# LuaAndC/lua-mapreduce-1

Hardware: AMD Instinct MI355X
Metric: words/sec (whole node), Europarl-v7 word-count 197 splits, 1/2/4/8 MI355X (higher is better)
Workload: dtype int64; 1 GPU; model=wordcount (MapReduce: taskfn/mapfn/partitionfn/reducefn), global_batch=197, seq_len=10000, parallelism=dp1, num_reducers=10, words=49158635, bytes=291393897, valid=True, input=host-staged-every-step

## Files before the change

csrc/hip/wordcount3.hip:

```cpp
#include <hip/hip_runtime.h>
#include "mr_common.h"
#include "hashtab.h"

MR_LONG_MASK_SYMBOL(wc3)

namespace mr {
namespace v3 {

constexpr int SEG = 16;
constexpr int PAD = 16;
constexpr int HALO = 64;
constexpr int PROBES = 32;

template <int T, int SLOTS>
struct Lds {
  static constexpr int TILE = T * SEG;
  static constexpr int STAGED = TILE + HALO;
  static constexpr int TXT = PAD + STAGED + 32;
  static constexpr int WSW = STAGED / 32 + 2;
  static constexpr int MAXTOK = T * 4;
  u8 txt[TXT];
  u32 ws[WSW];
  u16 tokpos[MAXTOK];
  u32 wsum[T / 64];
  u32 tnext;
  u64 tag[SLOTS];
  u32 cnt[SLOTS];
  u32 rep[SLOTS];
  u64 lo[SLOTS];
  u64 hi[SLOTS];
  u32 nclaimed;
};

struct Ovf {
  u64* hi;
  u64* lo;
  u64* rep;
  u64 cap;
  unsigned long long* counter;
};

__device__ __forceinline__ u32 ws_mask_word(u32 w) {
  u32 m = 0;
#pragma unroll
  for (int j = 0; j < 4; ++j) m |= (is_ws((w >> (8 * j)) & 0xFFu) ? 1u : 0u) << j;
  return m;
}

__device__ __forceinline__ u32 ws_mask16(uint4 q) {
  return ws_mask_word(q.x) | (ws_mask_word(q.y) << 4) | (ws_mask_word(q.z) << 8) | (ws_mask_word(q.w) << 12);
}

__device__ __forceinline__ u32 funnel(u32 a, u32 b, u32 r8) { return r8 ? ((a >> r8) | (b << (32 - r8))) : a; }

__device__ u64 long_lo_global(const u8* text, u64 p0, u64 len) {
  u64 h = long_hash_init(len);
  for (u64 w = 0; w < len; w += 8) {
    const u64 n = (len - w) < 8 ? (len - w) : 8;
    const u64 word = load_word_le(text + p0 + w, n);
    h = long_hash_step(h, word);
  }
  return long_lo(h, mr_long_mask);
}

__device__ __forceinline__ uint4 load16(const u8* __restrict__ text, u64 gpos, u64 nbytes, int aligned) {
  if (aligned && gpos + SEG <= nbytes) {
    typedef u32 v4u __attribute__((ext_vector_type(4)));
    const v4u v = __builtin_nontemporal_load(reinterpret_cast<const v4u*>(text + gpos));
    return make_uint4(v.x, v.y, v.z, v.w);
  }
  u32 w[4];
#pragma unroll
  for (int k = 0; k < 4; ++k) {
    w[k] = 0;
#pragma unroll
    for (int j = 0; j < 4; ++j) {
      const u64 p = gpos + 4 * k + j;
      w[k] |= (p < nbytes ? (u32)text[p] : 32u) << (8 * j);
    }
  }
  return make_uint4(w[0], w[1], w[2], w[3]);
}

template <int T, int SLOTS>
__device__ __forceinline__ bool lds_insert(Lds<T, SLOTS>& L, u64 hi, u64 lo, u32 rep, const u8* kb) {
  u64 h = hi ^ (lo * 0x9E3779B97F4A7C15ull);
  h ^= h >> 31;
  h *= 0xC2B2AE3D27D4EB4Full;
  h ^= h >> 29;
  const bool exact = (lo - 1 < 7) && (hi & 0xFFull) == 0;
  const u64 tag = exact ? (hi | lo) : ((h & ~0xFFull) | 0x80ull);
  u32 slot = (u32)(h >> 40) & (SLOTS - 1);
  constexpr u32 LIMIT = SLOTS * 3 / 4;
  for (int probes = 0; probes < PROBES;) {
    u64 cur = __hip_atomic_load(&L.tag[slot], __ATOMIC_RELAXED, __HIP_MEMORY_SCOPE_WORKGROUP);
    if (cur == 0) {
      if (__hip_atomic_load(&L.nclaimed, __ATOMIC_RELAXED, __HIP_MEMORY_SCOPE_WORKGROUP) >= LIMIT) return false;
      u64 expected = 0;
      if (__hip_atomic_compare_exchange_strong(&L.tag[slot], &expected, tag, __ATOMIC_RELAXED, __ATOMIC_RELAXED,
                                               __HIP_MEMORY_SCOPE_WORKGROUP)) {
        L.hi[slot] = hi;
        L.rep[slot] = rep;
        __hip_atomic_fetch_add(&L.cnt[slot], 1u, __ATOMIC_RELAXED, __HIP_MEMORY_SCOPE_WORKGROUP);
        __hip_atomic_fetch_add(&L.nclaimed, 1u, __ATOMIC_RELAXED, __HIP_MEMORY_SCOPE_WORKGROUP);
        if (exact) L.lo[slot] = lo;
        else __hip_atomic_store(&L.lo[slot], lo, __ATOMIC_RELEASE, __HIP_MEMORY_SCOPE_WORKGROUP);
        return true;
      }
      cur = expected;
    }
    if (cur == tag) {
      if (exact) {
        __hip_atomic_fetch_add(&L.cnt[slot], 1u, __ATOMIC_RELAXED, __HIP_MEMORY_SCOPE_WORKGROUP);
        return true;
      }
      const u64 l = __hip_atomic_load(&L.lo[slot], __ATOMIC_ACQUIRE, __HIP_MEMORY_SCOPE_WORKGROUP);
      if (l == 0) continue;
      if (l == lo && L.hi[slot] == hi &&
          (!key_is_long(lo) || rep_bytes_equal(kb, make_rep(L.rep[slot] & 0xFFFFu, L.rep[slot] >> 16),
                                               make_rep(rep & 0xFFFFu, rep >> 16)))) {
        __hip_atomic_fetch_add(&L.cnt[slot], 1u, __ATOMIC_RELAXED, __HIP_MEMORY_SCOPE_WORKGROUP);
        return true;
      }
    }
    slot = (slot + 1) & (SLOTS - 1);
    ++probes;
  }
  return false;
}

template <int T, int SLOTS, int TPC, bool STAMPS = false, bool DYN = false>
__global__ void __launch_bounds__(T) wc_map3_kernel(const u8* __restrict__ text, u64 nbytes, u64 rep_base, GTab g,
                                                    Ovf ovf, int aligned, u64* __restrict__ stamps = nullptr) {
  using L_t = Lds<T, SLOTS>;
  constexpr int TILE = L_t::TILE;
  constexpr int STAGED = L_t::STAGED;
  constexpr int WSW = L_t::WSW;
  constexpr u64 CHUNK = (u64)TILE * TPC;
  __shared__ __attribute__((aligned(16))) L_t L;
  const int t = threadIdx.x;
  const u64 chunk_begin = (u64)blockIdx.x * CHUNK;
  if (chunk_begin >= nbytes) return;
  const u64 chunk_end = min(chunk_begin + CHUNK, nbytes);
  [[maybe_unused]] u64 st_bar = 0, st_stage = 0, st_scan = 0, st_list = 0, st_loop = 0, st_flush = 0, st_p = 0;
  auto clk = [&]() -> u64 {
    if constexpr (STAMPS) return wall_clock64();
    return 0;
  };
  [[maybe_unused]] const u64 st_t0 = clk();
  auto bar = [&]() {
    const u64 a = clk();
    __syncthreads();
    if constexpr (STAMPS) st_bar += clk() - a;
  };
  for (int s = t; s < SLOTS; s += T) {
    L.tag[s] = 0;
    L.cnt[s] = 0;
    L.lo[s] = 0;
  }
  if (t == 0) {
    L.nclaimed = 0;
    L.txt[PAD - 1] = chunk_begin > 0 ? text[chunk_begin - 1] : (u8)' ';
    L.ws[WSW - 2] = 0xFFFFFFFFu;
    L.ws[WSW - 1] = 0xFFFFFFFFu;
  }
  u32 claims = 0;
  u16* ws16 = reinterpret_cast<u16*>(L.ws);
  const u32* txt32 = reinterpret_cast<const u32*>(L.txt);
  constexpr int NH = HALO / SEG;
  uint4 q = load16(text, chunk_begin + (u64)t * SEG, nbytes, aligned);
  uint4 qh = make_uint4(0, 0, 0, 0);
  if (t < NH) qh = load16(text, chunk_begin + TILE + (u64)t * SEG, nbytes, aligned);
  for (u64 tile_base = chunk_begin; tile_base < chunk_end; tile_base += TILE) {
    if (t == T - 1 && tile_base != chunk_begin) L.txt[PAD - 1] = L.txt[PAD + TILE - 1];
    bar();
    st_p = clk();
    *reinterpret_cast<uint4*>(L.txt + PAD + t * SEG) = q;
    ws16[t] = (u16)ws_mask16(q);
    if (t < NH) {
      *reinterpret_cast<uint4*>(L.txt + PAD + TILE + t * SEG) = qh;
      ws16[T + t] = (u16)ws_mask16(qh);
    }
    if constexpr (STAMPS) st_stage += clk() - st_p;
    bar();
    st_p = clk();
    const u64 next = tile_base + TILE;
    if (next < chunk_end) {
      q = load16(text, next + (u64)t * SEG, nbytes, aligned);
      if (t < NH) qh = load16(text, next + TILE + (u64)t * SEG, nbytes, aligned);
    }
    auto process = [&](u32 p) {
      u32 qq = p + 1;
      u32 wd = L.ws[qq >> 5] >> (qq & 31);
      u32 end;
      if (wd) {
        end = qq + __builtin_ctz(wd);
      } else {
        u32 k = (qq >> 5) + 1;
        while (L.ws[k] == 0) ++k;
        end = 32 * k + __builtin_ctz(L.ws[k]);
      }
      u64 len = end - p;
      const u64 gpos = tile_base + p;
      const u32 b = PAD + p;
      const u32 a = b >> 2;
      const u32 r8 = (b & 3u) * 8u;
      const u32 x0 = txt32[a], x1 = txt32[a + 1], x2 = txt32[a + 2], x3 = txt32[a + 3], x4 = txt32[a + 4];
      const u64 le_hi = (u64)funnel(x0, x1, r8) | ((u64)funnel(x1, x2, r8) << 32);
      const u64 le_lo = (u64)funnel(x2, x3, r8) | ((u64)funnel(x3, x4, r8) << 32);
      u64 hi = __builtin_bswap64(le_hi);
      u64 lo;
      if (end >= (u32)STAGED) {
        u64 pe = tile_base + STAGED;
        while (pe < nbytes && !is_ws(text[pe])) ++pe;
        len = pe - gpos;
      }
      if (len <= (u64)PACK_MAX) {
        if (len < 8) hi &= ~0ull << (8 * (8 - len));
        lo = len > 8 ? (__builtin_bswap64(le_lo) & (~0ull << (8 * (16 - len)))) : 0ull;
        lo |= len;
      } else {
        lo = long_lo_global(text, gpos, len);
      }
      const bool ok = len < 65536 && lds_insert(L, hi, lo, (u32)(gpos - chunk_begin) | ((u32)len << 16),
                                                 text + chunk_begin);
      if (!ok) {
        const u64 grep = make_rep(rep_base + gpos, len);
        const unsigned long long idx = atomicAdd(ovf.counter, 1ull);
        if (idx < ovf.cap) {
          ovf.hi[idx] = hi;
          ovf.lo[idx] = lo;
          ovf.rep[idx] = grep;
        } else {
          claims += gtab_insert(g, hi, lo, 1, grep, OP_SUM) == 2;
        }
      }
    };
    const u64 seg_base = tile_base + (u64)t * SEG;
    u32 starts = 0;
    if (seg_base < chunk_end) {
      const u32 m = ws16[t];
      const u32 prev_ws = t ? ((ws16[t - 1] >> 15) & 1u) : (is_ws(L.txt[PAD - 1]) ? 1u : 0u);
      starts = (~m) & ((m << 1) | prev_ws) & 0xFFFFu;
      const u64 lim_own = chunk_end - seg_base;
      if (lim_own < 16) starts &= (1u << lim_own) - 1u;
    }
    {
      constexpr int MAXTOK = L_t::MAXTOK;
      const int lane = t & 63, wave = t >> 6;
      const u32 c = __builtin_popcount(starts);
      u32 incl = c;
#pragma unroll
      for (int o = 1; o < 64; o <<= 1) {
        const u32 v = __shfl_up(incl, o);
        if (lane >= o) incl += v;
      }
      if (lane == 63) L.wsum[wave] = incl;
      if (DYN && t == 0) L.tnext = 0;
      if constexpr (STAMPS) st_scan += clk() - st_p;
      bar();
      st_p = clk();
      u32 base = 0, total = 0;
#pragma unroll
      for (int w = 0; w < T / 64; ++w) {
        const u32 x = L.wsum[w];
        base += w < wave ? x : 0u;
        total += x;
      }
      u32 k = base + incl - c;
      while (starts) {
        const int i = __builtin_ctz(starts);
        starts &= starts - 1;
        if (k < (u32)MAXTOK) L.tokpos[k] = (u16)(t * SEG + i);
        else process((u32)t * SEG + i);
        ++k;
      }
      if constexpr (STAMPS) st_list += clk() - st_p;
      bar();
      st_p = clk();
      const u32 ntok = total < (u32)MAXTOK ? total : (u32)MAXTOK;
      if constexpr (DYN) {
        for (;;) {
          u32 b0 = 0;
          if (lane == 0) b0 = __hip_atomic_fetch_add(&L.tnext, 64u, __ATOMIC_RELAXED, __HIP_MEMORY_SCOPE_WORKGROUP);
          b0 = __shfl(b0, 0);
          if (b0 >= ntok) break;
          if (b0 + lane < ntok) process(L.tokpos[b0 + lane]);
        }
      } else {
        for (u32 x = t; x < ntok; x += T) process(L.tokpos[x]);
      }
    }
    if constexpr (STAMPS) st_loop += clk() - st_p;
    bar();
  }
  [[maybe_unused]] const u64 st_f0 = clk();
  constexpr int PER = SLOTS / T;
  static_assert(SLOTS % T == 0, "slots must be a multiple of the block size");
  u64 khi[PER], klo[PER], ktag[PER], kslot[PER], gt[PER], gl[PER], gh[PER];
  u32 kcnt[PER], krep[PER];
#pragma unroll
  for (int k = 0; k < PER; ++k) {
    const int s = t + k * T;
    kcnt[k] = L.tag[s] != 0 ? L.cnt[s] : 0u;
    khi[k] = L.hi[s];
    klo[k] = L.lo[s];
    krep[k] = L.rep[s];
    ktag[k] = gtab_tag(khi[k], klo[k]);
    kslot[k] = gtab_home(ktag[k], g.mask);
  }
#pragma unroll
  for (int k = 0; k < PER; ++k) {
    if (kcnt[k]) {
      gt[k] = ld_agent(&g.s[kslot[k]].tag);
      if (!gtab_tag_exact(ktag[k])) {
        gl[k] = ld_agent(&g.s[kslot[k]].lo);
        gh[k] = ld_agent(&g.s[kslot[k]].hi);
      } else {
        gl[k] = klo[k];
        gh[k] = khi[k];
      }
    }
  }
  u32 state = 0;
#pragma unroll
  for (int k = 0; k < PER; ++k) {
    if (!kcnt[k]) {
      state |= 1u << k;
    } else if (gt[k] == ktag[k] && gl[k] == klo[k] && gh[k] == khi[k] && !key_is_long(klo[k])) {
      fold_value(&g.val[kslot[k]], (long long)kcnt[k], OP_SUM);
      state |= 1u << k;
    }
  }
  u32 won = 0;
#pragma unroll
  for (int k = 0; k < PER; ++k) {
    if (!(state & (1u << k)) && gt[k] == 0) {
      u64 expected = 0;
      if (__hip_atomic_compare_exchange_strong(&g.s[kslot[k]].tag, &expected, ktag[k], __ATOMIC_RELAXED,
                                               __ATOMIC_RELAXED, __HIP_MEMORY_SCOPE_AGENT))
        won |= 1u << k;
    }
  }
  if (won) {
#pragma unroll
    for (int k = 0; k < PER; ++k) {
      if (won & (1u << k)) {
        const u32 r = krep[k];
        st_agent(&g.s[kslot[k]].hi, khi[k]);
        st_agent(&g.s[kslot[k]].rep, make_rep(rep_base + chunk_begin + (r & 0xFFFFu), r >> 16));
        fold_value(&g.val[kslot[k]], (long long)kcnt[k], OP_SUM);
      }
    }
    asm volatile("s_waitcnt vmcnt(0)" ::: "memory");
#pragma unroll
    for (int k = 0; k < PER; ++k)
      if (won & (1u << k)) st_agent(&g.s[kslot[k]].lo, klo[k]);
    claims += __builtin_popcount(won);
    state |= won;
  }
#pragma unroll
  for (int k = 0; k < PER; ++k) {
    if (state & (1u << k)) continue;
    const u32 r = krep[k];
    claims += gtab_insert(g, khi[k], klo[k], (long long)kcnt[k],
                          make_rep(rep_base + chunk_begin + (r & 0xFFFFu), r >> 16), OP_SUM) == 2;
  }
  gtab_count_claims(g, claims);
  if constexpr (STAMPS) {
    const u64 now = clk();
    st_flush = now - st_f0;
    if ((t & 63) == 0) {
      u64* o = stamps + ((u64)blockIdx.x * (T / 64) + (t >> 6)) * 8;
      o[0] = now - st_t0;
      o[1] = st_bar;
      o[2] = st_stage;
      o[3] = st_scan;
      o[4] = st_list;
      o[5] = st_loop;
      o[6] = st_flush;
      o[7] = claims;
    }
  }
}

__global__ void __launch_bounds__(256) ovf_agg3_kernel(Ovf o, GTab g) {
  const unsigned long long n0 = *o.counter;
  const u64 n = n0 < o.cap ? n0 : o.cap;
  const u64 stride = (u64)gridDim.x * blockDim.x;
  u32 claims = 0;
  for (u64 i = (u64)blockIdx.x * blockDim.x + threadIdx.x; i < n; i += stride)
    claims += gtab_insert(g, o.hi[i], o.lo[i], 1ll, o.rep[i], OP_SUM) == 2;
  gtab_count_claims(g, claims);
}

constexpr int MAP_T = 512, MAP_SLOTS = 2048, MAP_TPC = 1;
static_assert(sizeof(Lds<MAP_T, MAP_SLOTS>) <= 80 * 1024, "two workgroups per CU");

static int g_map_dyn = 1;

template <int T, int SLOTS, int TPC>
static void launch_map3(const u8* text, u64 nbytes, u64 rep_base, const GTab& g, const Ovf& o, int aligned,
                        hipStream_t stream, u64* stamps = nullptr) {
  constexpr u64 CHUNK = (u64)T * SEG * TPC;
  const u64 nblocks = (nbytes + CHUNK - 1) / CHUNK;
  const dim3 grid((unsigned)nblocks), block(T);
  if (stamps && g_map_dyn)
    hipLaunchKernelGGL((wc_map3_kernel<T, SLOTS, TPC, true, true>), grid, block, 0, stream, text, nbytes, rep_base, g,
                       o, aligned, stamps);
  else if (stamps)
    hipLaunchKernelGGL((wc_map3_kernel<T, SLOTS, TPC, true>), grid, block, 0, stream, text, nbytes, rep_base, g, o,
                       aligned, stamps);
  else if (g_map_dyn)
    hipLaunchKernelGGL((wc_map3_kernel<T, SLOTS, TPC, false, true>), grid, block, 0, stream, text, nbytes, rep_base,
                       g, o, aligned, nullptr);
  else
    hipLaunchKernelGGL((wc_map3_kernel<T, SLOTS, TPC>), grid, block, 0, stream, text, nbytes, rep_base, g, o, aligned,
                       nullptr);
}

}
}

using namespace mr;

extern "C" {

int mr_wc3_set_dyn(int on) {
  v3::g_map_dyn = on ? 1 : 0;
  return 0;
}

int mr_wc_map3(const void* text, u64 nbytes, u64 rep_base, void* tag, void* hi, void* lo, void* val, void* rep,
               void* ctrl, u64 cap, void* ovf_hi, void* ovf_lo, void* ovf_rep, u64 ovf_cap, void* ovf_counter,
               hipStream_t stream) {
  if (nbytes == 0) return 0;
  (void)hi, (void)lo, (void)val;
  GTab g = gtab_make(tag, val, ctrl, cap, (const u8*)text - rep_base);
  v3::Ovf o{(u64*)ovf_hi, (u64*)ovf_lo, (u64*)ovf_rep, ovf_cap, (unsigned long long*)ovf_counter};
  const int aligned = ((uintptr_t)text & 15) == 0;
  const u8* t = (const u8*)text;
  v3::launch_map3<v3::MAP_T, v3::MAP_SLOTS, v3::MAP_TPC>(t, nbytes, rep_base, g, o, aligned, stream);
  hipLaunchKernelGGL(v3::ovf_agg3_kernel, dim3(1024), dim3(256), 0, stream, o, g);
  return (int)hipGetLastError();
}

int mr_wc_map3_stamped(const void* text, u64 nbytes, u64 rep_base, void* tag, void* val, void* ctrl, u64 cap,
                       void* ovf_hi, void* ovf_lo, void* ovf_rep, u64 ovf_cap, void* ovf_counter, void* stamps,
                       hipStream_t stream) {
  if (nbytes == 0 || stamps == nullptr) return nbytes ? -1 : 0;
  GTab g = gtab_make(tag, val, ctrl, cap, (const u8*)text - rep_base);
  v3::Ovf o{(u64*)ovf_hi, (u64*)ovf_lo, (u64*)ovf_rep, ovf_cap, (unsigned long long*)ovf_counter};
  const int aligned = ((uintptr_t)text & 15) == 0;
  v3::launch_map3<v3::MAP_T, v3::MAP_SLOTS, v3::MAP_TPC>((const u8*)text, nbytes, rep_base, g, o, aligned, stream,
                                                          (u64*)stamps);
  hipLaunchKernelGGL(v3::ovf_agg3_kernel, dim3(1024), dim3(256), 0, stream, o, g);
  return (int)hipGetLastError();
}

}
```

Before: 9.574 billion words/s.

## Streamline map kernel: SWAR whitespace mask, aligned loads, outlined cold paths

Replaces the per-byte whitespace test with a SWAR bit trick and always issues aligned 16-byte loads by shifting the base pointer back and blanking the leading and trailing bytes with spaces. Cold paths (long-token hashing, global insert, long-key compare) are moved into noinline functions, and the LDS insert is rewritten as a single-exit loop, both aimed at cutting register pressure and divergence. Short tokens now get their length from one alignbit of the whitespace bitmap. Exact-key slots store the key only in the tag, and token-list overflow is handled inside the processing loop. The aim is fewer instructions and VGPRs in the hot map loop, at the risk of call overhead and subtle edge-case bugs around the alignment lead.

```diff
diff --git a/csrc/hip/wordcount3.hip b/csrc/hip/wordcount3.hip
--- a/csrc/hip/wordcount3.hip
+++ b/csrc/hip/wordcount3.hip
@@ -41,10 +41,14 @@
 };
 
 __device__ __forceinline__ u32 ws_mask_word(u32 w) {
-  u32 m = 0;
-#pragma unroll
-  for (int j = 0; j < 4; ++j) m |= (is_ws((w >> (8 * j)) & 0xFFu) ? 1u : 0u) << j;
-  return m;
+  const u32 l7 = w & 0x7F7F7F7Fu;
+  const u32 ge9 = l7 + 0x77777777u;
+  const u32 ge14 = l7 + 0x72727272u;
+  const u32 ne32 = (l7 ^ 0x20202020u) + 0x7F7F7F7Fu;
+  u32 m = (((ge9 & ~ge14) | ~ne32) & ~w & 0x80808080u) >> 7;
+  m |= m >> 7;
+  m |= m >> 14;
+  return m & 0xFu;
 }
 
 __device__ __forceinline__ u32 ws_mask16(uint4 q) {
@@ -53,7 +57,7 @@
 
 __device__ __forceinline__ u32 funnel(u32 a, u32 b, u32 r8) { return r8 ? ((a >> r8) | (b << (32 - r8))) : a; }
 
-__device__ u64 long_lo_global(const u8* text, u64 p0, u64 len) {
+__device__ __noinline__ u64 long_lo_global(const u8* text, u64 p0, u64 len) {
   u64 h = long_hash_init(len);
   for (u64 w = 0; w < len; w += 8) {
     const u64 n = (len - w) < 8 ? (len - w) : 8;
@@ -63,23 +67,41 @@
   return long_lo(h, mr_long_mask);
 }
 
-__device__ __forceinline__ uint4 load16(const u8* __restrict__ text, u64 gpos, u64 nbytes, int aligned) {
-  if (aligned && gpos + SEG <= nbytes) {
-    typedef u32 v4u __attribute__((ext_vector_type(4)));
-    const v4u v = __builtin_nontemporal_load(reinterpret_cast<const v4u*>(text + gpos));
-    return make_uint4(v.x, v.y, v.z, v.w);
-  }
-  u32 w[4];
+__device__ __noinline__ u64 token_end_global(const u8* text, u64 pe, u64 end) {
+  while (pe < end && !is_ws(text[pe])) ++pe;
+  return pe;
+}
+
+__device__ __noinline__ bool lds_long_equal(const u8* kb, u32 ra, u32 rb) {
+  return rep_bytes_equal(kb, make_rep(ra & 0xFFFFu, ra >> 16), make_rep(rb & 0xFFFFu, rb >> 16));
+}
+
+__device__ __noinline__ u32 gtab_insert_sum(GTab g, u64 hi, u64 lo, u32 cnt, u64 rep) {
+  return gtab_insert(g, hi, lo, (long long)cnt, rep, OP_SUM) == 2;
+}
+
+__device__ __noinline__ uint4 space_out16(uint4 q, u32 from, u32 to) {
+  u32 w[4] = {q.x, q.y, q.z, q.w};
 #pragma unroll
   for (int k = 0; k < 4; ++k) {
-    w[k] = 0;
-#pragma unroll
-    for (int j = 0; j < 4; ++j) {
-      const u64 p = gpos + 4 * k + j;
-      w[k] |= (p < nbytes ? (u32)text[p] : 32u) << (8 * j);
-    }
+    u32 keep = 0;
+#pragma unroll
+    for (int j = 0; j < 4; ++j) keep |= ((u32)(4 * k + j) >= from && (u32)(4 * k + j) < to) ? 0xFFu << (8 * j) : 0u;
+    w[k] = (w[k] & keep) | (0x20202020u & ~keep);
   }
   return make_uint4(w[0], w[1], w[2], w[3]);
+}
+
+__device__ __forceinline__ uint4 load16(const u8* __restrict__ text, u64 g, u32 lead, u64 end) {
+  if (g >= end) return make_uint4(0x20202020u, 0x20202020u, 0x20202020u, 0x20202020u);
+  typedef u32 v4u __attribute__((ext_vector_type(4)));
+  const v4u v = __builtin_nontemporal_load(reinterpret_cast<const v4u*>(text + g));
+  uint4 q = make_uint4(v.x, v.y, v.z, v.w);
+  const u32 from = g == 0 ? lead : 0u;
+  const u64 left = end - g;
+  if (__builtin_expect(from != 0 || left < (u64)SEG, 0))
+    q = space_out16(q, from, left < (u64)SEG ? (u32)left : (u32)SEG);
+  return q;
 }
 
 template <int T, int SLOTS>
@@ -92,46 +114,47 @@
   const u64 tag = exact ? (hi | lo) : ((h & ~0xFFull) | 0x80ull);
   u32 slot = (u32)(h >> 40) & (SLOTS - 1);
   constexpr u32 LIMIT = SLOTS * 3 / 4;
-  for (int probes = 0; probes < PROBES;) {
+  bool ok = false, full = false;
+  u32 probes = 0;
+  do {
     u64 cur = __hip_atomic_load(&L.tag[slot], __ATOMIC_RELAXED, __HIP_MEMORY_SCOPE_WORKGROUP);
     if (cur == 0) {
-      if (__hip_atomic_load(&L.nclaimed, __ATOMIC_RELAXED, __HIP_MEMORY_SCOPE_WORKGROUP) >= LIMIT) return false;
-      u64 expected = 0;
-      if (__hip_atomic_compare_exchange_strong(&L.tag[slot], &expected, tag, __ATOMIC_RELAXED, __ATOMIC_RELAXED,
-                                               __HIP_MEMORY_SCOPE_WORKGROUP)) {
-        L.hi[slot] = hi;
-        L.rep[slot] = rep;
-        __hip_atomic_fetch_add(&L.cnt[slot], 1u, __ATOMIC_RELAXED, __HIP_MEMORY_SCOPE_WORKGROUP);
-        __hip_atomic_fetch_add(&L.nclaimed, 1u, __ATOMIC_RELAXED, __HIP_MEMORY_SCOPE_WORKGROUP);
-        if (exact) L.lo[slot] = lo;
-        else __hip_atomic_store(&L.lo[slot], lo, __ATOMIC_RELEASE, __HIP_MEMORY_SCOPE_WORKGROUP);
-        return true;
-      }
-      cur = expected;
-    }
+      full = __hip_atomic_load(&L.nclaimed, __ATOMIC_RELAXED, __HIP_MEMORY_SCOPE_WORKGROUP) >= LIMIT;
+      if (!full) {
+        u64 expected = 0;
+        ok = __hip_atomic_compare_exchange_strong(&L.tag[slot], &expected, tag, __ATOMIC_RELAXED, __ATOMIC_RELAXED,
+                                                  __HIP_MEMORY_SCOPE_WORKGROUP);
+        cur = expected;
+        if (ok) {
+          L.rep[slot] = rep;
+          __hip_atomic_fetch_add(&L.nclaimed, 1u, __ATOMIC_RELAXED, __HIP_MEMORY_SCOPE_WORKGROUP);
+          if (!exact) {
+            L.hi[slot] = hi;
+            __hip_atomic_store(&L.lo[slot], lo, __ATOMIC_RELEASE, __HIP_MEMORY_SCOPE_WORKGROUP);
+          }
+        }
+      }
+    }
+    bool wait = false;
     if (cur == tag) {
-      if (exact) {
-        __hip_atomic_fetch_add(&L.cnt[slot], 1u, __ATOMIC_RELAXED, __HIP_MEMORY_SCOPE_WORKGROUP);
-        return true;
-      }
-      const u64 l = __hip_atomic_load(&L.lo[slot], __ATOMIC_ACQUIRE, __HIP_MEMORY_SCOPE_WORKGROUP);
-      if (l == 0) continue;
-      if (l == lo && L.hi[slot] == hi &&
-          (!key_is_long(lo) || rep_bytes_equal(kb, make_rep(L.rep[slot] & 0xFFFFu, L.rep[slot] >> 16),
-                                               make_rep(rep & 0xFFFFu, rep >> 16)))) {
-        __hip_atomic_fetch_add(&L.cnt[slot], 1u, __ATOMIC_RELAXED, __HIP_MEMORY_SCOPE_WORKGROUP);
-        return true;
-      }
-    }
-    slot = (slot + 1) & (SLOTS - 1);
-    ++probes;
-  }
-  return false;
+      ok = exact;
+      if (!exact) {
+        const u64 l = __hip_atomic_load(&L.lo[slot], __ATOMIC_ACQUIRE, __HIP_MEMORY_SCOPE_WORKGROUP);
+        wait = l == 0;
+        ok = l == lo && L.hi[slot] == hi && (!key_is_long(lo) || lds_long_equal(kb, L.rep[slot], rep));
+      }
+    }
+    if (ok) __hip_atomic_fetch_add(&L.cnt[slot], 1u, __ATOMIC_RELAXED, __HIP_MEMORY_SCOPE_WORKGROUP);
+    const u32 adv = (ok || full || wait) ? 0u : 1u;
+    slot = (slot + adv) & (SLOTS - 1);
+    probes += adv;
+  } while (!ok && !full && probes < (u32)PROBES);
+  return ok;
 }
 
 template <int T, int SLOTS, int TPC, bool STAMPS = false, bool DYN = false>
 __global__ void __launch_bounds__(T) wc_map3_kernel(const u8* __restrict__ text, u64 nbytes, u64 rep_base, GTab g,
-                                                    Ovf ovf, int aligned, u64* __restrict__ stamps = nullptr) {
+                                                    Ovf ovf, u32 lead, u64* __restrict__ stamps = nullptr) {
   using L_t = Lds<T, SLOTS>;
   constexpr int TILE = L_t::TILE;
   constexpr int STAGED = L_t::STAGED;
@@ -168,9 +191,9 @@
   u16* ws16 = reinterpret_cast<u16*>(L.ws);
   const u32* txt32 = reinterpret_cast<const u32*>(L.txt);
   constexpr int NH = HALO / SEG;
-  uint4 q = load16(text, chunk_begin + (u64)t * SEG, nbytes, aligned);
+  uint4 q = load16(text, chunk_begin + (u64)t * SEG, lead, nbytes);
   uint4 qh = make_uint4(0, 0, 0, 0);
-  if (t < NH) qh = load16(text, chunk_begin + TILE + (u64)t * SEG, nbytes, aligned);
+  if (t < NH) qh = load16(text, chunk_begin + TILE + (u64)t * SEG, lead, nbytes);
   for (u64 tile_base = chunk_begin; tile_base < chunk_end; tile_base += TILE) {
     if (t == T - 1 && tile_base != chunk_begin) L.txt[PAD - 1] = L.txt[PAD + TILE - 1];
     bar();
@@ -186,21 +209,12 @@
     st_p = clk();
     const u64 next = tile_base + TILE;
     if (next < chunk_end) {
-      q = load16(text, next + (u64)t * SEG, nbytes, aligned);
-      if (t < NH) qh = load16(text, next + TILE + (u64)t * SEG, nbytes, aligned);
+      q = load16(text, next + (u64)t * SEG, lead, nbytes);
+      if (t < NH) qh = load16(text, next + TILE + (u64)t * SEG, lead, nbytes);
     }
     auto process = [&](u32 p) {
-      u32 qq = p + 1;
-      u32 wd = L.ws[qq >> 5] >> (qq & 31);
-      u32 end;
-      if (wd) {
-        end = qq + __builtin_ctz(wd);
-      } else {
-        u32 k = (qq >> 5) + 1;
-        while (L.ws[k] == 0) ++k;
-        end = 32 * k + __builtin_ctz(L.ws[k]);
-      }
-      u64 len = end - p;
+      const u32 qq = p + 1;
+      const u32 wd = __builtin_amdgcn_alignbit(L.ws[(qq >> 5) + 1], L.ws[qq >> 5], qq & 31u);
       const u64 gpos = tile_base + p;
       const u32 b = PAD + p;
       const u32 a = b >> 2;
@@ -210,21 +224,27 @@
       const u64 le_lo = (u64)funnel(x2, x3, r8) | ((u64)funnel(x3, x4, r8) << 32);
       u64 hi = __builtin_bswap64(le_hi);
       u64 lo;
-      if (end >= (u32)STAGED) {
-        u64 pe = tile_base + STAGED;
-        while (pe < nbytes && !is_ws(text[pe])) ++pe;
-        len = pe - gpos;
-      }
-      if (len <= (u64)PACK_MAX) {
-        if (len < 8) hi &= ~0ull << (8 * (8 - len));
-        lo = len > 8 ? (__builtin_bswap64(le_lo) & (~0ull << (8 * (16 - len)))) : 0ull;
-        lo |= len;
+      u64 len;
+      if (__builtin_expect((wd & 0x7FFFu) != 0, 1)) {
+        const u32 n = 1u + (u32)__builtin_ctz(wd);
+        len = n;
+        hi &= ~0ull << (n < 8 ? 8 * (8 - n) : 0);
+        lo = (n > 8 ? (__builtin_bswap64(le_lo) & (~0ull << (8 * ((16 - n) & 7u)))) : 0ull) | n;
       } else {
+        u32 end;
+        if (wd) {
+          end = qq + __builtin_ctz(wd);
+        } else {
+          u32 k = (qq >> 5) + 1;
+          while (L.ws[k] == 0) ++k;
+          end = 32 * k + __builtin_ctz(L.ws[k]);
+        }
+        len = end >= (u32)STAGED ? token_end_global(text, tile_base + STAGED, nbytes) - gpos : (u64)(end - p);
         lo = long_lo_global(text, gpos, len);
       }
       const bool ok = len < 65536 && lds_insert(L, hi, lo, (u32)(gpos - chunk_begin) | ((u32)len << 16),
                                                  text + chunk_begin);
-      if (!ok) {
+      if (__builtin_expect(!ok, 0)) {
         const u64 grep = make_rep(rep_base + gpos, len);
         const unsigned long long idx = atomicAdd(ovf.counter, 1ull);
         if (idx < ovf.cap) {
@@ -232,7 +252,7 @@
           ovf.lo[idx] = lo;
           ovf.rep[idx] = grep;
         } else {
-          claims += gtab_insert(g, hi, lo, 1, grep, OP_SUM) == 2;
+          claims += gtab_insert_sum(g, hi, lo, 1u, grep);
         }
       }
     };
@@ -267,28 +287,38 @@
         base += w < wave ? x : 0u;
         total += x;
       }
-      u32 k = base + incl - c;
-      while (starts) {
-        const int i = __builtin_ctz(starts);
+      for (u32 k = base + incl - c; starts && k < (u32)MAXTOK; ++k) {
+        L.tokpos[k] = (u16)(t * SEG + __builtin_ctz(starts));
         starts &= starts - 1;
-        if (k < (u32)MAXTOK) L.tokpos[k] = (u16)(t * SEG + i);
-        else process((u32)t * SEG + i);
-        ++k;
       }
       if constexpr (STAMPS) st_list += clk() - st_p;
       bar();
       st_p = clk();
       const u32 ntok = total < (u32)MAXTOK ? total : (u32)MAXTOK;
-      if constexpr (DYN) {
-        for (;;) {
-          u32 b0 = 0;
-          if (lane == 0) b0 = __hip_atomic_fetch_add(&L.tnext, 64u, __ATOMIC_RELAXED, __HIP_MEMORY_SCOPE_WORKGROUP);
-          b0 = __shfl(b0, 0);
-          if (b0 >= ntok) break;
-          if (b0 + lane < ntok) process(L.tokpos[b0 + lane]);
+      constexpr u32 NONE = 0xFFFFFFFFu;
+      bool listed = true;
+      for (u32 x = t;;) {
+        u32 p = NONE;
+        if (listed) {
+          if constexpr (DYN) {
+            u32 b0 = 0;
+            if (lane == 0)
+              b0 = __hip_atomic_fetch_add(&L.tnext, 64u, __ATOMIC_RELAXED, __HIP_MEMORY_SCOPE_WORKGROUP);
+            b0 = __builtin_amdgcn_readfirstlane(b0);
+            if (b0 >= ntok) listed = false;
+            else if (b0 + lane < ntok) p = L.tokpos[b0 + lane];
+          } else {
+            if (x >= ntok) listed = false;
+            else p = L.tokpos[x];
+            x += T;
+          }
         }
-      } else {
-        for (u32 x = t; x < ntok; x += T) process(L.tokpos[x]);
+        if (!listed) {
+          if (!starts) break;
+          p = (u32)t * SEG + __builtin_ctz(starts);
+          starts &= starts - 1;
+        }
+        if (p != NONE) process(p);
       }
     }
     if constexpr (STAMPS) st_loop += clk() - st_p;
@@ -302,9 +332,11 @@
 #pragma unroll
   for (int k = 0; k < PER; ++k) {
     const int s = t + k * T;
-    kcnt[k] = L.tag[s] != 0 ? L.cnt[s] : 0u;
-    khi[k] = L.hi[s];
-    klo[k] = L.lo[s];
+    const u64 ltag = L.tag[s];
+    const bool ex = gtab_tag_exact(ltag);
+    kcnt[k] = ltag != 0 ? L.cnt[s] : 0u;
+    khi[k] = ex ? ltag & ~0xFFull : L.hi[s];
+    klo[k] = ex ? ltag & 0xFFull : L.lo[s];
     krep[k] = L.rep[s];
     ktag[k] = gtab_tag(khi[k], klo[k]);
     kslot[k] = gtab_home(ktag[k], g.mask);
@@ -359,18 +391,19 @@
     claims += __builtin_popcount(won);
     state |= won;
   }
-#pragma unroll
-  for (int k = 0; k < PER; ++k) {
-    if (state & (1u << k)) continue;
-    const u32 r = krep[k];
-    claims += gtab_insert(g, khi[k], klo[k], (long long)kcnt[k],
-                          make_rep(rep_base + chunk_begin + (r & 0xFFFFu), r >> 16), OP_SUM) == 2;
+  for (u32 rest = ~state & ((1u << PER) - 1u); rest; rest &= rest - 1) {
+    const int s = t + __builtin_ctz(rest) * T;
+    const u32 r = L.rep[s];
+    const u64 ltag = L.tag[s];
+    const bool ex = gtab_tag_exact(ltag);
+    claims += gtab_insert_sum(g, ex ? ltag & ~0xFFull : L.hi[s], ex ? ltag & 0xFFull : L.lo[s], L.cnt[s],
+                              make_rep(rep_base + chunk_begin + (r & 0xFFFFu), r >> 16));
   }
   gtab_count_claims(g, claims);
   if constexpr (STAMPS) {
     const u64 now = clk();
     st_flush = now - st_f0;
-    if ((t & 63) == 0) {
+    if ((t & 63) == 0 && chunk_begin + lead < nbytes) {
       u64* o = stamps + ((u64)blockIdx.x * (T / 64) + (t >> 6)) * 8;
       o[0] = now - st_t0;
       o[1] = st_bar;
@@ -400,22 +433,25 @@
 static int g_map_dyn = 1;
 
 template <int T, int SLOTS, int TPC>
-static void launch_map3(const u8* text, u64 nbytes, u64 rep_base, const GTab& g, const Ovf& o, int aligned,
-                        hipStream_t stream, u64* stamps = nullptr) {
+static void launch_map3(const u8* text0, u64 nbytes0, u64 rep_base0, const GTab& g, const Ovf& o, hipStream_t stream,
+                        u64* stamps = nullptr) {
   constexpr u64 CHUNK = (u64)T * SEG * TPC;
+  const u32 lead = (u32)((uintptr_t)text0 & 15u);
+  const u8* text = text0 - lead;
+  const u64 nbytes = nbytes0 + lead, rep_base = rep_base0 - lead;
   const u64 nblocks = (nbytes + CHUNK - 1) / CHUNK;
   const dim3 grid((unsigned)nblocks), block(T);
   if (stamps && g_map_dyn)
     hipLaunchKernelGGL((wc_map3_kernel<T, SLOTS, TPC, true, true>), grid, block, 0, stream, text, nbytes, rep_base, g,
-                       o, aligned, stamps);
+                       o, lead, stamps);
   else if (stamps)
     hipLaunchKernelGGL((wc_map3_kernel<T, SLOTS, TPC, true>), grid, block, 0, stream, text, nbytes, rep_base, g, o,
-                       aligned, stamps);
+                       lead, stamps);
   else if (g_map_dyn)
     hipLaunchKernelGGL((wc_map3_kernel<T, SLOTS, TPC, false, true>), grid, block, 0, stream, text, nbytes, rep_base,
-                       g, o, aligned, nullptr);
+                       g, o, lead, nullptr);
   else
-    hipLaunchKernelGGL((wc_map3_kernel<T, SLOTS, TPC>), grid, block, 0, stream, text, nbytes, rep_base, g, o, aligned,
+    hipLaunchKernelGGL((wc_map3_kernel<T, SLOTS, TPC>), grid, block, 0, stream, text, nbytes, rep_base, g, o, lead,
                        nullptr);
 }
 
@@ -438,9 +474,7 @@
   (void)hi, (void)lo, (void)val;
   GTab g = gtab_make(tag, val, ctrl, cap, (const u8*)text - rep_base);
   v3::Ovf o{(u64*)ovf_hi, (u64*)ovf_lo, (u64*)ovf_rep, ovf_cap, (unsigned long long*)ovf_counter};
-  const int aligned = ((uintptr_t)text & 15) == 0;
-  const u8* t = (const u8*)text;
-  v3::launch_map3<v3::MAP_T, v3::MAP_SLOTS, v3::MAP_TPC>(t, nbytes, rep_base, g, o, aligned, stream);
+  v3::launch_map3<v3::MAP_T, v3::MAP_SLOTS, v3::MAP_TPC>((const u8*)text, nbytes, rep_base, g, o, stream);
   hipLaunchKernelGGL(v3::ovf_agg3_kernel, dim3(1024), dim3(256), 0, stream, o, g);
   return (int)hipGetLastError();
 }
@@ -451,9 +485,7 @@
   if (nbytes == 0 || stamps == nullptr) return nbytes ? -1 : 0;
   GTab g = gtab_make(tag, val, ctrl, cap, (const u8*)text - rep_base);
   v3::Ovf o{(u64*)ovf_hi, (u64*)ovf_lo, (u64*)ovf_rep, ovf_cap, (unsigned long long*)ovf_counter};
-  const int aligned = ((uintptr_t)text & 15) == 0;
-  v3::launch_map3<v3::MAP_T, v3::MAP_SLOTS, v3::MAP_TPC>((const u8*)text, nbytes, rep_base, g, o, aligned, stream,
-                                                          (u64*)stamps);
+  v3::launch_map3<v3::MAP_T, v3::MAP_SLOTS, v3::MAP_TPC>((const u8*)text, nbytes, rep_base, g, o, stream, (u64*)stamps);
   hipLaunchKernelGGL(v3::ovf_agg3_kernel, dim3(1024), dim3(256), 0, stream, o, g);
   return (int)hipGetLastError();
 }
```

After: 9.577 billion words/s (median of 3 runs). About the same (+0.0%).
